# Leo-Li009/fs-dkr

Hardware: AMD Instinct MI355X
Metric: collect() proofs verified/sec at n=64, 2048-bit N; 4096-bit modexp/s/GPU (higher is better)
Workload: dtype u32 (radix-2^29 digits, u64 accumulators); 1 GPU; RefreshMessage::collect n=64 t=32: 60 refresh + 4 JoinMessage, M=256, 2048-bit N (BASELINE configs[2]); one step = the whole collect() call (pack, pre-pass + upload, pipeline, first error, key updates, share recovery); n=64, t=32, refresh=60, joins=4, parallelism=refresh messages sharded over 1 GPU(s)

## Files before the change

### fs-dkr_amd/csrc/capi.cpp

```cpp
#include "fsdkr/fsdkr.h"

#include <hip/hip_runtime.h>

#include <cstdarg>
#include <cstdio>
#include <cstdlib>
#include <cstring>
#include <algorithm>
#include <atomic>
#include <map>
#include <condition_variable>
#include <mutex>
#include <thread>
#include <string>
#include <vector>

#include "ctx.hpp"
#include "kernels.h"
#include "verify.h"

using namespace fsdkr;

namespace fsdkr {

// ... 280 lines not shown
  if (count == 0) return FSDKR_OK;
  uint32_t grp = c->modexp_group ? c->modexp_group : group;
  if (grp == kWideGroup && (group != kWideGroup || k32 != 128)) grp = 16;
  if (grp == kWaveGroup && k32 != 128) grp = 16;
  if (c->ct) grp = 0;
  const bool slide_shape = k32 == 128 ? (grp == 4 || grp == 8 || grp == 16 || grp == kWideGroup)
                                      : (k32 == 192 && grp == 8 && split && split->lo_bit && !split->nadic);
  const bool slide = (desc_flags & kDescSlide) && (desc_flags & kDescOutIdx) && !c->ct && grp == group && slide_shape;
  const int KD = table_digits(k32, grp);
  if (!KD) {
    c->fail("unsupported modulus width %u limbs", k32);
    return FSDKR_E_UNSUPPORTED;
  }
  const uint32_t ebits = exp_bits ? exp_bits : 1;
  const bool nadic = split && split->lo_bit && split->nadic;
  const uint32_t w = nadic ? kNadicWindow : slide ? choose_slide_window(ebits) : choose_window(ebits);
  const uint32_t nwin = (ebits + w - 1) / w;
  const size_t entries = slide ? ((size_t)1 << (w - 1)) + 1 : (size_t)1 << w;
  uint32_t* d_table = (uint32_t*)c->buf(table_tag, sizeof(uint32_t) * (size_t)count * entries * KD);
  if (!d_table) {
    c->fail("device allocation failed (%u instances, window %u)", count, w);
    return FSDKR_E_OOM;
  }
  const size_t n8 = (size_t)count * 8, n4 = (size_t)count * 4;
  ModexpArgs a;
  a.base_ptr = reinterpret_cast<const uint64_t*>(d_desc);
  a.exp_ptr = reinterpret_cast<const uint64_t*>(d_desc + n8);
  a.base_len = reinterpret_cast<const uint32_t*>(d_desc + 2 * n8);
  a.exp_len = reinterpret_cast<const uint32_t*>(d_desc + 2 * n8 + n4);
  a.mod_idx = reinterpret_cast<const uint32_t*>(d_desc + 2 * n8 + 2 * n4);
  a.nwin_i = reinterpret_cast<const uint32_t*>(d_desc + 2 * n8 + 3 * n4);
  a.nwin = nwin;
  a.window = w;
  a.consts = d_consts;
  a.out = d_out;
  a.table = d_table;
  a.count = count;
  a.prio = prio;
  a.group = grp;
  a.ct = c->ct ? 1u : 0u;
  a.slide = slide ? 1u : 0u;
  a.out_idx = (desc_flags & kDescOutIdx) ? reinterpret_cast<const uint32_t*>(d_desc + 2 * n8 + 4 * n4) : nullptr;
  if (split && split->lo_bit) {
    if (!slide || grp != group || !(grp == 4 || grp == 8 || grp == 16 || grp == kWideGroup)) {
      c->fail("split chains need the 4 / 8 / 16 / 32-lane sliding-window shapes, 8 lanes at 192 limbs (group %u)", grp);
      return FSDKR_E_ARG;
    }
    const std::string base(table_tag);
    if (nadic && grp != 16) {
      c->fail("the N-adic head needs the 16-lane shape (group %u)", grp);
      return FSDKR_E_ARG;
    }
    a.nadic = split->nadic;
    a.lo_bit = split->lo_bit;
    a.tail = split->tail ? 1u : 0u;
    a.state = (uint32_t*)c->buf((base + "_state").c_str(), (size_t)count * KD * 4);
    if (!a.state) {
      c->fail("device allocation failed (split chain state)");
      return FSDKR_E_OOM;
    }
    if (split->tail && split->d_desc2) {
      a.base2_ptr = reinterpret_cast<const uint64_t*>(split->d_desc2);
      a.exp2_ptr = reinterpret_cast<const uint64_t*>(split->d_desc2 + n8);
      a.exp2_len = reinterpret_cast<const uint32_t*>(split->d_desc2 + 2 * n8);
      a.table2 = (uint32_t*)c->buf((base + "_t2").c_str(), (size_t)count * 16 * KD * 4);
      if (!a.table2) {
        c->fail("device allocation failed (joint table)");
        return FSDKR_E_OOM;
      }
      if (split->d_desc3) {
        a.base3_ptr = reinterpret_cast<const uint64_t*>(split->d_desc3);
        a.exp3_ptr = reinterpret_cast<const uint64_t*>(split->d_desc3 + n8);
        a.exp3_len = reinterpret_cast<const uint32_t*>(split->d_desc3 + 2 * n8);
        a.exp3_bits = split->exp3_bits;
        a.table3 = (uint32_t*)c->buf((base + "_t3").c_str(), (size_t)count * 16 * KD * 4);
        if (!a.table3) {
          c->fail("device allocation failed (joint table)");
          return FSDKR_E_OOM;
        }
      }
    }
  }
  const size_t tm = c->tbeg("modexp", st);
  int rc = c->hip_check(modexp(k32, a, st), "modexp launch");
  c->tend(tm, st);
  return rc;
}

void ModexpJob::pack(std::vector<uint8_t>& dst) const {
  const size_t n8 = size() * 8, n4 = size() * 4;
  const size_t o = dst.size();
  dst.resize(o + desc_bytes());
  memcpy(dst.data() + o, base_ptr.data(), n8);
  memcpy(dst.data() + o + n8, exp_ptr.data(), n8);
  memcpy(dst.data() + o + 2 * n8, base_len.data(), n4);
  memcpy(dst.data() + o + 2 * n8 + n4, exp_len.data(), n4);
  memcpy(dst.data() + o + 2 * n8 + 2 * n4, mod_idx.data(), n4);
  const uint32_t w = choose_window(exp_bits ? exp_bits : 1);
  uint32_t* nw = reinterpret_cast<uint32_t*>(dst.data() + o + 2 * n8 + 3 * n4);
  for (size_t k = 0; k < size(); ++k) nw[k] = ebits[k] ? (ebits[k] + w - 1) / w : 1u;
  if (!out_idx.empty()) memcpy(dst.data() + o + 2 * n8 + 4 * n4, out_idx.data(), n4);
}

int launch_modexp_job(Ctx* c, const ModexpJob& job, const uint32_t* d_consts, uint32_t* d_out, const char* tag,
                      uint32_t group, uint32_t desc_flags) {
  const uint32_t count = (uint32_t)job.size();
// ... 432 lines not shown
```

### fs-dkr_amd/csrc/collect_prestart.cpp

```cpp
#include "collect.hpp"

namespace fsdkr {

void nadic_consts(const uint32_t* N, uint32_t nl, uint32_t* out) {
  constexpr uint32_t kM29 = (1u << 29) - 1;
  auto digits = [&](const hbn::Limbs& v, uint32_t* dst, int nd) {
    for (int j = 0; j < nd; ++j) {
      const size_t bit = 29u * (size_t)j, w = bit >> 5, sh = bit & 31;
      const uint64_t lo = w < v.size() ? v[w] : 0u, hi = w + 1 < v.size() ? v[w + 1] : 0u;
      dst[j] = (uint32_t)(((hi << 32) | lo) >> sh) & kM29;
    }
  };
  std::fill(out, out + kNadicStride, 0u);
  const hbn::Limbs n = hbn::from(N, nl);
  uint32_t inv = N[0];
  for (int it = 0; it < 5; ++it) inv *= 2u - N[0] * inv;
  const uint32_t k0 = (0u - inv) & kM29;
  const hbn::Limbs Np = hbn::mul(n, hbn::Limbs{k0});
  const hbn::Limbs one{1u};
  hbn::Limbs q, r;
  hbn::divmod_knuth(hbn::mod(hbn::shl(one, 2 * 29 * 72), hbn::mul(Np, Np)), Np, &q, &r);
  const hbn::Limbs nq = q.empty() ? hbn::Limbs{} : hbn::sub(Np, q);
  const hbn::Limbs NN = hbn::mul(n, n);
  const hbn::Limbs C1 = hbn::mod(hbn::shl(one, 3 * 29 * 72), NN);
  const hbn::Limbs C2 = hbn::mod(hbn::mul(hbn::sub(NN, hbn::mod(Np, NN)), C1), NN);
  digits(Np, out + kNadicNp, 72);
  digits(r, out + kNadicR0, 72);
  digits(nq, out + kNadicR1, 72);
  digits(C1, out + kNadicC1, 144);
  digits(C2, out + kNadicC2, 144);
}


static int prestart_fb_tables(Ctx* c, const fsdkr_collect_batch* bs, uint32_t count, GaPre& g, uint32_t n, uint32_t P) {
  if (g.sess.size() != count) return FSDKR_OK;
  const uint32_t M = bs[0].m_security;
  bool exact_s = true, exact_z = true;
  uint32_t nl = 0, Mt = 0, s1l = 0, s3l = 0, zl = 0;
  for (uint32_t k = 0; k < count; ++k) {
    const fsdkr_collect_batch* b = bs + k;
    if (!b->recv_ntilde || !b->recv_h1 || !b->recv_h2 || !b->s1l || !b->s3l || !b->ped_T || !b->ped_N || !b->zl ||
        !b->m_security || b->m_security != M)
      return FSDKR_OK;
    exact_s = exact_s && b->pdl_s1 && b->pdl_s3 && b->rp_s1 && b->rp_s2;
    exact_z = exact_z && b->ped_Z;
    nl = std::max(nl, b->nl);
    Mt += b->n_refresh + b->n_join;
    s1l = std::max(s1l, b->s1l);
    s3l = std::max(s3l, b->s3l);
    zl = std::max(zl, b->zl);
    for (uint32_t i = 0; i < g.sess[k].n; ++i)
      if (!is_odd(b->recv_ntilde + (size_t)i * b->nl)) return FSDKR_OK;
  }
  uint32_t bh1 = 1, bh2 = 1, bz = 1;
  if (exact_s) {
    for (uint32_t k = 0; k < count; ++k) {
      const fsdkr_collect_batch* b = bs + k;
      for (size_t p = 0; p < (size_t)g.sess[k].R * g.sess[k].n; ++p) {
        bh1 = std::max(bh1, std::max(hbn::bitlen(b->pdl_s1 + p * b->s1l, b->s1l), hbn::bitlen(b->rp_s1 + p * b->s1l, b->s1l)));
        bh2 = std::max(bh2, std::max(hbn::bitlen(b->pdl_s3 + p * b->s3l, b->s3l), hbn::bitlen(b->rp_s2 + p * b->s3l, b->s3l)));
      }
    }
  } else {
    bh1 = 32 * s1l;
    bh2 = 32 * s3l;
  }
  if (exact_z) {
    for (uint32_t k = 0; k < count; ++k) {
      const fsdkr_collect_batch* b = bs + k;
      const size_t rows = (size_t)(b->n_refresh + b->n_join) * M;
      for (size_t q = 0; q < rows; ++q) bz = std::max(bz, hbn::bitlen(b->ped_Z + q * b->zl, b->zl));
    }
  } else {
    bz = 32 * zl;
  }
  const uint32_t w = fb_window(std::max(std::max(bh1, bh2), bz));
  const FbLayout L = fb_layout(n, Mt, w, bh1, bh2, bz);
  const uint32_t nb = 2 * n + Mt, entries = L.entries, nmod = n + Mt;
  const int KD = shape_digits(nl);
  std::vector<uint32_t> bbits(nb), bcnt(nb, M);
  for (uint32_t r = 0; r < n; ++r) {
    bbits[r] = bh1;
    bbits[n + Mt + r] = bh2;
// ... 672 lines not shown
```

### fs-dkr_amd/csrc/kernels.h

```cpp
#pragma once
#include <hip/hip_runtime.h>
#include <stdint.h>

namespace fsdkr {

constexpr int BLOCK = 256;

constexpr int cons_stride(int kd) { return 6 * kd + 8; }
constexpr int cons_scaled(int kd) { return 3 * kd + 4; }
constexpr bool scaled_ok(int kd, int k32) { return 32 * k32 + 31 <= 29 * kd; }

struct ModexpArgs {
  const uint64_t* base_ptr;
  const uint32_t* base_len;
  const uint64_t* exp_ptr;
  const uint32_t* exp_len;
  uint32_t nwin;
  uint32_t window;
  const uint32_t* nwin_i;
  const uint32_t* mod_idx;
  const uint32_t* consts;
  uint32_t* out;
  uint32_t* table;
  uint32_t count;
  uint32_t prio;
  uint32_t group;
  uint32_t ct;
  uint32_t slide;
  const uint32_t* out_idx;
  uint32_t lo_bit = 0;
  uint32_t tail = 0;
  uint32_t* state = nullptr;
  const uint64_t* base2_ptr = nullptr;
  const uint64_t* exp2_ptr = nullptr;
  const uint32_t* exp2_len = nullptr;
  uint32_t* table2 = nullptr;
  const uint32_t* nadic = nullptr;
  const uint64_t* base3_ptr = nullptr;
  const uint64_t* exp3_ptr = nullptr;
  const uint32_t* exp3_len = nullptr;
  uint32_t* table3 = nullptr;
  uint32_t exp3_bits = 0;
};

constexpr int kNadicNp = 0, kNadicR0 = 72, kNadicR1 = 144, kNadicC1 = 216, kNadicC2 = 360, kNadicStride = 512;
constexpr uint32_t kNadicWindow = 7;

int shape_digits(uint32_t k32);
constexpr uint32_t kWideGroup = 32;
constexpr uint32_t kWaveGroup = 64;
int shape_digits_g(uint32_t k32, uint32_t group);
int table_digits(uint32_t k32, uint32_t group);
hipError_t mod_setup(uint32_t k32, const uint32_t* mods, uint32_t n_mod, uint32_t* consts, hipStream_t st);
hipError_t mod_setup_wave(uint32_t k32, const uint32_t* mods, uint32_t n_mod, uint32_t* consts, hipStream_t st);
hipError_t mod_setup_g(uint32_t k32, uint32_t group, const uint32_t* mods, uint32_t n_mod, uint32_t* consts,
                       hipStream_t st);
hipError_t modexp(uint32_t k32, const ModexpArgs& a, hipStream_t st);

struct MrTailArgs {
  const uint32_t* x;
  const uint32_t* consts;
  const uint32_t* s;
  uint32_t s_max;
  uint32_t* verdict;
  uint32_t count;
};
constexpr uint32_t kPrimeLimbs = 32;
hipError_t mr_tail(uint32_t k32, const MrTailArgs& a, hipStream_t st);

}
```

### fs-dkr_amd/csrc/modexp.hip

```cpp
#include "mont29.hpp"
#include "kernels.h"
#include <cstdlib>
#include <initializer_list>

namespace fsdkr {

template <int KD, int G, int K32>
__global__ __launch_bounds__(BLOCK) void mod_setup_kernel(const uint32_t* __restrict__ mods, uint32_t n_mod,
                                                          uint32_t* __restrict__ consts) {
  using MT = Mont29<KD, G>;
  constexpr int L = MT::L;
  constexpr int IPB = BLOCK / G;
  constexpr bool SC = scaled_ok(KD, K32);
  __shared__ uint32_t lds[IPB * KD];
  const int g = threadIdx.x % G;
  const int li = threadIdx.x / G;
  const uint32_t mi = blockIdx.x * IPB + li;
  if (mi >= (SC ? 2 * n_mod : n_mod)) return;
  const bool scaled = SC && mi >= n_mod;
  const uint32_t m = scaled ? mi - n_mod : mi;
  __builtin_amdgcn_s_setprio(3);
  uint32_t* stream = lds + li * KD;
  const uint32_t* N = mods + (size_t)m * K32;
  MT M;
// ... 398 lines not shown
  constexpr int IPB = BLOCK / G;
  __shared__ uint32_t lds[IPB * KD];
  const int g = threadIdx.x % G;
  const int li = threadIdx.x / G;
  const uint32_t inst = blockIdx.x * (blockDim.x / G) + li;
  if (inst >= a.count) return;
  if (a.prio == 1) __builtin_amdgcn_s_setprio(1);
  else if (a.prio == 2) __builtin_amdgcn_s_setprio(2);
  else if (a.prio >= 3) __builtin_amdgcn_s_setprio(3);
  uint32_t* stream = lds + li * KD;
  const uint32_t* C = a.nadic + (size_t)a.mod_idx[inst] * kNadicStride;
  const bool hi = g >= 8;
  uint32_t sh_hi = hi ? 1u : 0u, m_hi = hi ? 0xFFFFFFFFu : 0u;
  asm volatile("" : "+v"(sh_hi), "+v"(m_hi));
  MT M;
  M.init_pair(g);
#pragma unroll
  for (int j = 0; j < L; ++j) M.n[j] = C[kNadicNp + (g & 7) * L + j];
  M.ninv = 1u;
  const uint32_t tw = 1u << (kNadicWindow - 1);
  uint32_t* T = a.table + (size_t)inst * (tw + 1) * KD;
  const uint64_t ea = a.exp_ptr[inst];
  const uint32_t* E = reinterpret_cast<const uint32_t*>(
      ((uint64_t)(uint32_t)__builtin_amdgcn_readfirstlane((int)(uint32_t)(ea >> 32)) << 32) |
      (uint32_t)__builtin_amdgcn_readfirstlane((int)(uint32_t)ea));
  const int exp_limbs = __builtin_amdgcn_readfirstlane((int)a.exp_len[inst]);
  auto bit = [&](int i) -> uint32_t { return (E[i >> 5] >> (i & 31)) & 1u; };
  int top = 32 * exp_limbs - 1;
  while (top >= 0 && E[top >> 5] == 0) top = (top & ~31) - 1;
  while (top >= 0 && !bit(top)) --top;
  const int lo = (int)a.lo_bit;
  auto window = [&](int i, int* jl) -> uint32_t {
    int j = max(i - (int)kNadicWindow + 1, lo);
    while (!bit(j)) ++j;
    uint32_t d = 0;
    for (int k = i; k >= j; --k) d = (d << 1) | bit(k);
    *jl = j;
    return d;
  };
  uint32_t acc[L];
#pragma unroll
  for (int j = 0; j < L; ++j) acc[j] = 0u;
  const uint32_t* B = reinterpret_cast<const uint32_t*>(a.base_ptr[inst]);
  const int blen = (int)min(a.base_len[inst], 64u);
  auto load = [&](const uint32_t* row) {
#pragma unroll
    for (int j = 0; j < L; ++j) acc[j] = row[g * L + j];
  };
  auto store = [&](uint32_t* row) {
#pragma unroll
    for (int j = 0; j < L; ++j) row[g * L + j] = acc[j];
  };
  const bool none = top < lo;
  {
    uint32_t b[L];
    __builtin_amdgcn_wave_barrier();
#pragma unroll
    for (int j = 0; j < L; ++j) {
      const int d = g * L + j;
      b[j] = C[kNadicR0 + d];
      if (!hi) stream[d] = none ? (d == 0 ? 1u : 0u) : digit_of(B, blen, d);
    }
    __builtin_amdgcn_wave_barrier();
    M.product_pair(acc, b, stream);
  }
  auto square = [&]() {
    __builtin_amdgcn_wave_barrier();
    lds_put<KD, G>(stream, acc, g);
    __builtin_amdgcn_wave_barrier();
    uint32_t b[L];
#pragma unroll
    for (int j = 0; j < L; ++j) b[j] = acc[j] << sh_hi;
    M.product_pair(acc, b, stream);
  };
  if (!none) {
    store(T);
    square();
    store(T + (size_t)tw * KD);
    load(T);
    int phase = tw > 1 ? 2 : 3, i = top, pend_mul = -1;
    uint32_t jt = 1, pend_sq = 0;
    for (;;) {
      if (phase == 3) {
        if (i == top) {
          int jl;
          const uint32_t d = window(i, &jl);
          load(T + (size_t)(d >> 1) * KD);
          i = jl - 1;
        }
        if (pend_sq == 0 && pend_mul < 0)
          while (i >= lo && !bit(i)) {
            ++pend_sq;
            --i;
          }
        for (; pend_sq; --pend_sq) square();
      }
      const uint32_t* src;
      if (phase == 2) {
        src = T + (size_t)tw * KD;
      } else if (pend_mul >= 0) {
        src = T + (size_t)pend_mul * KD;
        pend_mul = -1;
      } else if (i < lo) {
        break;
      } else {
        int jl;
        const uint32_t d = window(i, &jl);
        pend_sq = (uint32_t)(i - jl + 1);
        pend_mul = (int)(d >> 1);
        i = jl - 1;
        continue;
      }
      uint32_t y[L];
      __builtin_amdgcn_wave_barrier();
#pragma unroll
      for (int j = 0; j < L; ++j) y[j] = src[g * L + j];
      if (!hi) {
#pragma unroll
        for (int j = 0; j < L; ++j) {
          stream[g * L + j] = y[j];
          stream[72 + g * L + j] = acc[j];
        }
      }
#pragma unroll
      for (int j = 0; j < L; ++j) y[j] &= m_hi;
      __builtin_amdgcn_wave_barrier();
      M.product_pair2(acc, acc, y, stream, stream + 72);
      if (phase == 2) {
        store(T + (size_t)jt * KD);
        if (++jt == tw) phase = 3;
      }
    }
  }
#pragma unroll
  for (int j = 0; j < L; ++j) a.state[(size_t)inst * KD + g * L + j] = acc[j];
}

template <int KD, int G, int K32, bool QS, bool NA = false, bool J3 = false>
__global__ __launch_bounds__(BLOCK, 2) void modexp_tail_kernel(const ModexpArgs a) {
  using MT = Mont29<KD, G>;
  constexpr int L = MT::L;
  constexpr int IPB = BLOCK / G;
  constexpr int STRIDE = cons_stride(KD);
  static_assert(!QS || scaled_ok(KD, K32), "quotient-scaled chains: N' within R/4");
  __shared__ uint32_t lds[IPB * KD];
  const int g = threadIdx.x % G;
  const int li = threadIdx.x / G;
  const uint32_t inst = blockIdx.x * (blockDim.x / G) + li;
  if (inst >= a.count) return;
  if (a.prio == 1) __builtin_amdgcn_s_setprio(1);
  else if (a.prio == 2) __builtin_amdgcn_s_setprio(2);
  else if (a.prio >= 3) __builtin_amdgcn_s_setprio(3);
  uint32_t* stream = lds + li * KD;
  const uint32_t* C0 = a.consts + (size_t)a.mod_idx[inst] * STRIDE;
  const uint32_t* C = QS ? C0 + cons_scaled(KD) : C0;
  MT M;
  M.init_lane(g);
#pragma unroll
  for (int j = 0; j < L; ++j) M.n[j] = C[g * L + j];
  M.ninv = C[3 * KD];
  auto mulx = [&](uint32_t* x) {
    if constexpr (QS) M.mul_s(x, x, stream);
    else M.mul(x, x, stream);
  };
  const uint32_t w = a.window, tw = 1u << (w - 1);
  uint32_t* T = a.table + (size_t)inst * (tw + 1) * KD;
  const uint64_t ea = a.exp_ptr[inst];
  const uint32_t* E = reinterpret_cast<const uint32_t*>(
      ((uint64_t)(uint32_t)__builtin_amdgcn_readfirstlane((int)(uint32_t)(ea >> 32)) << 32) |
      (uint32_t)__builtin_amdgcn_readfirstlane((int)(uint32_t)ea));
  const int exp_limbs = __builtin_amdgcn_readfirstlane((int)a.exp_len[inst]);
  auto bit = [&](int i) -> uint32_t { return (i >> 5) < exp_limbs ? (E[i >> 5] >> (i & 31)) & 1u : 0u; };
  const int lo = (int)a.lo_bit;
  constexpr bool ACC_LATE = K32 > 128;
  static_assert(!(ACC_LATE && NA), "the N-adic entry converts the accumulator first");
  uint32_t acc[L];
  if constexpr (!ACC_LATE) {
#pragma unroll
    for (int j = 0; j < L; ++j) acc[j] = a.state[(size_t)inst * KD + g * L + j];
  }
  auto put_row = [&](const uint32_t* row) {
    __builtin_amdgcn_wave_barrier();
#pragma unroll
    for (int j = 0; j < L; ++j) stream[g * L + j] = row[g * L + j];
// ... 123 lines not shown
      pend_d = d;
    }
    __builtin_amdgcn_wave_barrier();
    lds_put<KD, G>(stream, acc, g);
    __builtin_amdgcn_wave_barrier();
    if constexpr (QS) M.sqr_s(acc, acc, stream);
    else M.sqr(acc, acc, stream);
    if (!NA && i == pend_at) {
      put_row(T + (size_t)(pend_d >> 1) * KD);
      mulx(acc);
      pend_at = -1;
    }
    if (NA && (i & 3) == 0) {
      const uint32_t d = (i >> 5) < exp_limbs ? (E[i >> 5] >> (i & 31)) & 15u : 0u;
      if (d) {
        put_row(T + (size_t)d * KD);
        mulx(acc);
      }
    }
    if (joint && (i & 3) == 0) {
      put_row(T2 + (size_t)((ew >> (i & 31)) & 15u) * KD);
      mulx(acc);
    }
    if constexpr (J3) {
      if ((i & 3) == 0 && i < e3bits) {
        put_row(T3 + (size_t)((ew3 >> (i & 31)) & 15u) * KD);
        mulx(acc);
      }
    }
  }
  if constexpr (QS) {
    const uint32_t* CX = C0;
    if constexpr (ACC_LATE) asm volatile("" : "+v"(CX) : "v"(acc[0]));
#pragma unroll
    for (int j = 0; j < L; ++j) M.n[j] = CX[g * L + j];
    M.ninv = CX[3 * KD];
  }
  __builtin_amdgcn_wave_barrier();
#pragma unroll
  for (int j = 0; j < L; ++j) stream[g * L + j] = (g == 0 && j == 0) ? 1u : 0u;
  __builtin_amdgcn_wave_barrier();
  M.mul(acc, acc, stream);
  M.carry_exact(acc);
  M.sub_if_ge(acc);
  __builtin_amdgcn_wave_barrier();
  lds_put<KD, G>(stream, acc, g);
  __builtin_amdgcn_wave_barrier();
  uint32_t* O = a.out + (size_t)(a.out_idx ? a.out_idx[inst] : inst) * K32;
  constexpr int LO = K32 / G;
#pragma unroll
  for (int k = 0; k < LO; ++k) O[g * LO + k] = limb_of(stream, KD, g * LO + k);
}

template <int KR, int L, int K32>
__global__ __launch_bounds__(64) void modexp_wave_kernel(const ModexpArgs a) {
  constexpr int KD = 64 * L;
  using MT = Mont29<KD, 64, KR>;
  constexpr int STRIDE = cons_stride(KR);
  __shared__ uint32_t lds[KD];
  const int g = threadIdx.x;
  const uint32_t inst = blockIdx.x;
  if (inst >= a.count) return;
  if (a.prio == 1) __builtin_amdgcn_s_setprio(1);
  else if (a.prio == 2) __builtin_amdgcn_s_setprio(2);
  else if (a.prio >= 3) __builtin_amdgcn_s_setprio(3);
  const uint32_t* C = a.consts + (size_t)a.mod_idx[inst] * STRIDE;
  const bool live = g * L < KR;
  MT M;
  M.init_lane(g);
#pragma unroll
  for (int j = 0; j < L; ++j) M.n[j] = live ? C[g * L + j] : 0u;
  M.ninv = (uint32_t)__builtin_amdgcn_readfirstlane((int)C[3 * KR]);
  const uint32_t w = a.window;
  const uint32_t tsize = 1u << w;
  uint32_t* T = a.table + (size_t)inst * tsize * KD;
  const uint32_t* E = reinterpret_cast<const uint32_t*>(a.exp_ptr[inst]);
  const uint32_t exp_limbs = a.exp_len[inst];
  uint32_t acc[L], opnd[L];
  const uint32_t* B = reinterpret_cast<const uint32_t*>(a.base_ptr[inst]);
  const int blen = (int)min(a.base_len[inst], (uint32_t)K32);
#pragma unroll
  for (int j = 0; j < L; ++j) acc[j] = digit_of(B, blen, g * L + j);
#pragma unroll
  for (int j = 0; j < L; ++j) T[g * L + j] = live ? C[KR + g * L + j] : 0u;
  const uint32_t nwin = a.nwin_i ? max(1u, a.nwin_i[inst]) : a.nwin;
  auto digit = [&](uint32_t k) -> uint32_t {
    const uint32_t p = (nwin - 1 - k) * w;
    const uint32_t lo = p >> 5, sh = p & 31;
    const uint32_t v0 = (lo < exp_limbs) ? E[lo] : 0u;
    const uint32_t v1 = (lo + 1 < exp_limbs) ? E[lo + 1] : 0u;
    return (uint32_t)(mk64(v0, v1) >> sh) & (tsize - 1);
  };
  const uint32_t n_build = tsize - 1;
  const uint32_t n_steps = n_build + (nwin - 1) * (w + 1) + 1;
  uint32_t k = 1, sub = 0;
  for (uint32_t st = 0; st < n_steps; ++st) {
    if (st == n_build) {
      const uint32_t d0 = digit(0);
#pragma unroll
      for (int j = 0; j < L; ++j) acc[j] = T[(size_t)d0 * KD + g * L + j];
    }
    if (st >= n_build && st < n_steps - 1 && sub < w) {
      M.sqr_w(acc, acc);
    } else {
      const uint32_t* src = (st == 0) ? nullptr : (st < n_build) ? T + KD : (st == n_steps - 1) ? nullptr
                                                                            : T + (size_t)digit(k) * KD;
// ... 22 lines not shown
  __builtin_amdgcn_wave_barrier();
  uint32_t* O = a.out + (size_t)(a.out_idx ? a.out_idx[inst] : inst) * K32;
  for (int q = g; q < K32; q += 64) O[q] = limb_of(lds, KR, q);
}

template <int KR, int L, int K32>
static hipError_t launch_setup_wave(const uint32_t* mods, uint32_t n_mod, uint32_t* consts, hipStream_t st) {
  const uint32_t waves = scaled_ok(KR, K32) ? 2 * n_mod : n_mod;
  if (waves == 0) return hipSuccess;
  hipLaunchKernelGGL((mod_setup_wave_kernel<KR, L, K32>), dim3(waves), dim3(64), 0, st, mods, n_mod, consts);
  return hipGetLastError();
}
template <int KD, int G, int K32>
static hipError_t launch_setup(const uint32_t* mods, uint32_t n_mod, uint32_t* consts, hipStream_t st) {
  constexpr int IPB = BLOCK / G;
  const uint32_t inst = scaled_ok(KD, K32) ? 2 * n_mod : n_mod;
  const uint32_t blocks = (inst + IPB - 1) / IPB;
  if (blocks == 0) return hipSuccess;
  hipLaunchKernelGGL((mod_setup_kernel<KD, G, K32>), dim3(blocks), dim3(BLOCK), 0, st, mods, n_mod, consts);
  return hipGetLastError();
}
constexpr uint32_t kSmallLaunchLanes = 256u * 4u * 64u;
static inline uint32_t block_threads(uint32_t lanes) { return lanes <= kSmallLaunchLanes ? 64u : (uint32_t)BLOCK; }

template <int KD, int G, int K32, bool CT = false, bool QS = false>
static hipError_t launch_modexp(const ModexpArgs& a, hipStream_t st) {
  const uint32_t bs = block_threads(a.count * G);
  const uint32_t ipb = bs / G;
  const uint32_t blocks = (a.count + ipb - 1) / ipb;
  if (blocks == 0) return hipSuccess;
  hipLaunchKernelGGL((modexp_kernel<KD, G, K32, CT, QS>), dim3(blocks), dim3(bs), 0, st, a);
  return hipGetLastError();
}

template <int KD, int G, int K32, bool QS>
static hipError_t launch_modexp_slide(const ModexpArgs& a, hipStream_t st) {
  const uint32_t bs = block_threads(a.count * G);
  const uint32_t ipb = bs / G;
  const uint32_t blocks = (a.count + ipb - 1) / ipb;
  if (blocks == 0) return hipSuccess;
  hipLaunchKernelGGL((modexp_slide_kernel<KD, G, K32, QS>), dim3(blocks), dim3(bs), 0, st, a);
  return hipGetLastError();
}

static hipError_t launch_modexp_nadic_head(const ModexpArgs& a, hipStream_t st) {
  const uint32_t bs = block_threads(a.count * 16);
  const uint32_t ipb = bs / 16;
  const uint32_t blocks = (a.count + ipb - 1) / ipb;
  if (blocks == 0) return hipSuccess;
  hipLaunchKernelGGL(modexp_nadic_head_kernel, dim3(blocks), dim3(bs), 0, st, a);
  return hipGetLastError();
}

template <int KD, int G, int K32, bool QS, bool NA = false, bool J3 = false>
static hipError_t launch_modexp_tail(const ModexpArgs& a, hipStream_t st) {
  const uint32_t bs = block_threads(a.count * G);
  const uint32_t ipb = bs / G;
  const uint32_t blocks = (a.count + ipb - 1) / ipb;
  if (blocks == 0) return hipSuccess;
  hipLaunchKernelGGL((modexp_tail_kernel<KD, G, K32, QS, NA, J3>), dim3(blocks), dim3(bs), 0, st, a);
  return hipGetLastError();
}

template <int KR, int L, int K32>
static hipError_t launch_modexp_wave(const ModexpArgs& a, hipStream_t st) {
  if (a.count == 0) return hipSuccess;
  hipLaunchKernelGGL((modexp_wave_kernel<KR, L, K32>), dim3(a.count), dim3(64), 0, st, a);
  return hipGetLastError();
}

hipError_t mod_setup_wave(uint32_t k32, const uint32_t* mods, uint32_t n_mod, uint32_t* consts, hipStream_t st) {
  if (k32 == 96) return launch_setup_wave<108, 2, 96>(mods, n_mod, consts, st);
  return mod_setup(k32, mods, n_mod, consts, st);
}

int shape_digits(uint32_t k32) {
  switch (k32) {
    case 64: return 72;
    case 96: return 108;
    case 128: return 144;
    case 192: return 216;
    default: return 0;
  }
}

int shape_digits_g(uint32_t k32, uint32_t group) {
  if (k32 == kPrimeLimbs) return 36;
  return (k32 == 128 && group == kWideGroup) ? 160 : shape_digits(k32);
}

int table_digits(uint32_t k32, uint32_t group) {
  if (k32 == 128 && group == kWaveGroup) return 192;
  return shape_digits_g(k32, group);
}

hipError_t mod_setup_g(uint32_t k32, uint32_t group, const uint32_t* mods, uint32_t n_mod, uint32_t* consts,
                       hipStream_t st) {
  if (k32 == 128 && group == kWideGroup) return launch_setup<160, 8, 128>(mods, n_mod, consts, st);
  return mod_setup(k32, mods, n_mod, consts, st);
}

hipError_t mod_setup(uint32_t k32, const uint32_t* mods, uint32_t n_mod, uint32_t* consts, hipStream_t st) {
  switch (k32) {
    case 32: return launch_setup<36, 2, 32>(mods, n_mod, consts, st);
    case 64: return launch_setup<72, 8, 64>(mods, n_mod, consts, st);
    case 96: return launch_setup<108, 4, 96>(mods, n_mod, consts, st);
// ... 7 lines not shown
  for (int g : allowed)
    if (g == forced) return g;
  constexpr uint64_t kLaneCapacity = 256ull * 4 * 3 * 64;
  int best = min_auto;
  for (int g : allowed)
    if (g > best && (uint64_t)count * (uint64_t)g <= kLaneCapacity) best = g;
  return best;
}

hipError_t modexp(uint32_t k32, const ModexpArgs& a, hipStream_t st) {
  if (a.ct) {
    if (a.group == kWideGroup) return hipErrorInvalidValue;
    switch (k32) {
      case 32: return launch_modexp<36, 4, 32, true>(a, st);
      case 64: return launch_modexp<72, 8, 64, true>(a, st);
      case 96: return launch_modexp<108, 4, 96, true>(a, st);
      case 128: return launch_modexp<144, 8, 128, true>(a, st);
      case 192: return launch_modexp<216, 8, 192, true>(a, st);
      default: return hipErrorInvalidValue;
    }
  }
  if (a.slide && k32 == 192) {
    if (a.ct || a.group != 8 || !a.lo_bit || a.nadic || !a.state) return hipErrorInvalidValue;
    if (!a.tail) return launch_modexp_slide<216, 8, 192, true>(a, st);
    if (a.base3_ptr) {
      if (!a.base2_ptr || !a.exp3_ptr || !a.exp3_len || !a.table3 || (a.exp3_bits & 3u) || a.exp3_bits > a.lo_bit)
        return hipErrorInvalidValue;
      return launch_modexp_tail<216, 8, 192, true, false, true>(a, st);
    }
    return launch_modexp_tail<216, 8, 192, true>(a, st);
  }
  if (a.slide) {
    if (k32 != 128 || a.ct || a.group == kWaveGroup) return hipErrorInvalidValue;
    if (a.base3_ptr) {
      if (!a.lo_bit || !a.tail || a.nadic || !a.base2_ptr || !a.exp3_ptr || !a.exp3_len || !a.table3 ||
          (a.exp3_bits & 3u) || a.exp3_bits > a.lo_bit)
        return hipErrorInvalidValue;
      switch (a.group) {
        case kWideGroup: return launch_modexp_tail<160, 32, 128, true, false, true>(a, st);
        case 16: return launch_modexp_tail<144, 16, 128, true, false, true>(a, st);
        case 8: return launch_modexp_tail<144, 8, 128, true, false, true>(a, st);
        case 4: return launch_modexp_tail<144, 4, 128, true, false, true>(a, st);
        default: return hipErrorInvalidValue;
      }
    }
    if (a.group == kWideGroup) {
      if (a.lo_bit && a.tail)
        return launch_modexp_tail<160, 32, 128, true>(a, st);
      return launch_modexp_slide<160, 32, 128, true>(a, st);
    }
    if (a.lo_bit) {
      if (a.nadic) {
        if (a.group != 16 || a.window != kNadicWindow || !a.state) return hipErrorInvalidValue;
        return a.tail ? launch_modexp_tail<144, 16, 128, true, true>(a, st) : launch_modexp_nadic_head(a, st);
      }
      switch (a.group) {
        case 16: return a.tail ? launch_modexp_tail<144, 16, 128, true>(a, st)
                               : launch_modexp_slide<144, 16, 128, true>(a, st);
        case 8: return a.tail ? launch_modexp_tail<144, 8, 128, true>(a, st)
                              : launch_modexp_slide<144, 8, 128, true>(a, st);
        case 4: return a.tail ? launch_modexp_tail<144, 4, 128, true>(a, st)
                              : launch_modexp_slide<144, 4, 128, true>(a, st);
        default: return hipErrorInvalidValue;
      }
    }
    switch (pick_group(a.count, (int)a.group, {4, 8, 16}, 4)) {
      case 16: return launch_modexp_slide<144, 16, 128, true>(a, st);
      case 8: return launch_modexp_slide<144, 8, 128, true>(a, st);
      default: return launch_modexp_slide<144, 4, 128, true>(a, st);
    }
  }
  switch (k32) {
    case 32:
      return pick_group(a.count, (int)a.group, {2, 4}, 4) == 2 ? launch_modexp<36, 2, 32>(a, st)
                                                              : launch_modexp<36, 4, 32>(a, st);
    case 64:
      switch (pick_group(a.count, (int)a.group, {2, 4, 8}, 4)) {
        case 8: return launch_modexp<72, 8, 64, false, true>(a, st);
        case 4: return launch_modexp<72, 4, 64, false, true>(a, st);
        default: return launch_modexp<72, 2, 64>(a, st);
      }
    case 96: return launch_modexp<108, 4, 96, false, true>(a, st);
    case 128:
      if (a.group == kWideGroup)
        return launch_modexp<160, 32, 128, false, true>(a, st);
      if (a.group == kWaveGroup) return launch_modexp_wave<144, 3, 128>(a, st);
      switch (pick_group(a.count, (int)a.group, {4, 8, 16}, 4)) {
        case 16: return launch_modexp<144, 16, 128, false, true>(a, st);
        case 8: return launch_modexp<144, 8, 128, false, true>(a, st);
        default: return launch_modexp<144, 4, 128, false, true>(a, st);
      }
    case 192:
      if (pick_group(a.count, (int)a.group, {4, 8}, 4) == 8)
        return launch_modexp<216, 8, 192, false, true>(a, st);
      return launch_modexp<216, 4, 192, false, true>(a, st);
    default: return hipErrorInvalidValue;
  }
}

}
```

### fs-dkr_amd/fsdkr/_native.py

```python
import ctypes
import os

import numpy as np

_HERE = os.path.dirname(os.path.abspath(__file__))
LIB_PATH = os.environ.get("FSDKR_LIB") or os.path.join(_HERE, "libfsdkr.so")

FSDKR_OK = 0
FSDKR_E_ARG = -1
FSDKR_E_HIP = -2
FSDKR_E_OOM = -3
FSDKR_E_UNSUPPORTED = -4
FSDKR_CFG_TIMING = 1
FSDKR_CFG_FB_BGMW = 2
FSDKR_CFG_FB_COMB = 4
FSDKR_CFG_INV_EACH = 8
FSDKR_CFG_GA_FULLWIDTH = 16

u32p = ctypes.POINTER(ctypes.c_uint32)


class FsdkrError(RuntimeError):
    def __init__(self, code, msg):
        super().__init__(f"fsdkr error {code}: {msg}")
        self.code = code


class _Cfg(ctypes.Structure):
    _fields_ = [("device", ctypes.c_int32), ("flags", ctypes.c_uint32)]


class CollectBatchC(ctypes.Structure):
    _fields_ = [(f, ctypes.c_uint32) for f in ("n_refresh", "n_join", "t", "m_security", "key_bits", "nl",
                                               "s1l", "s3l", "el", "zl", "yl")] + \
               [(f, u32p) for f in ("party_index", "msg_lens", "recv_n", "recv_ntilde", "recv_h1", "recv_h2",
                                    "enc", "commit", "pdl_z", "pdl_u3", "pdl_s2", "pdl_u1", "pdl_u2", "pdl_s1",
                                    "pdl_s3", "rp_z", "rp_s", "rp_e", "rp_s1", "rp_s2", "vss", "ped_S", "ped_T",
                                    "ped_N", "ped_A", "ped_Z", "ck_n", "ck_sigma", "dlog_N", "dlog_g", "dlog_ni",
                                    "dlog_x1", "dlog_x2", "dlog_y1", "dlog_y2")] + [("n_recv", ctypes.c_uint32)] + \
               [("vss_len", u32p), ("range_lens", u32p), ("ckl", ctypes.c_uint32), ("recv_avail", ctypes.c_uint32),
                ("ped_lens", u32p), ("ck_lens", u32p), ("pdl_s3_neg", ctypes.POINTER(ctypes.c_uint8)),
                ("neg_bits", ctypes.POINTER(ctypes.c_uint8)), ("ped_a_neg", ctypes.POINTER(ctypes.c_uint8))]


u8p = ctypes.POINTER(ctypes.c_uint8)


class VerdictsC(ctypes.Structure):
    _fields_ = [(f, u8p) for f in ("feldman", "pdl", "range", "ped", "ck", "dlog")] + \
               [(f, ctypes.c_uint32) for f in ("cap_pairs", "cap_msgs", "cap_joins")]


class BobBatchC(ctypes.Structure):
    _fields_ = [(f, ctypes.c_uint32) for f in ("count", "n_keys", "nl", "el", "s1l", "s2l", "t1l", "t2l")] + \
               [(f, u32p) for f in ("N", "Ntilde", "h1", "h2", "key_idx", "a_enc", "mta", "z", "t", "s", "e",
                                    "s1", "s2", "t1", "t2", "X", "u")]


class RecoverJobC(ctypes.Structure):
    _fields_ = [("nl", ctypes.c_uint32), ("t_vss", ctypes.c_uint32), ("t_key", ctypes.c_uint32),
                ("n_new", ctypes.c_uint32), ("old_index", u32p), ("cts", u32p), ("p", u32p), ("q", u32p),
                ("points", u32p), ("flags", ctypes.c_uint32)]


class RecoveredC(ctypes.Structure):
    _fields_ = [("share", ctypes.c_uint32 * 8), ("y", ctypes.c_uint32 * 16), ("pk_vec", u32p),
                ("status", ctypes.c_int32)]


def _struct_dtype(cls):
# ... 630 lines not shown
```

### include/fsdkr/fsdkr.h

```cpp
#ifndef FSDKR_FSDKR_H
#define FSDKR_FSDKR_H

#include <stdint.h>

#ifdef __cplusplus
extern "C" {
#endif

#define FSDKR_OK 0
#define FSDKR_E_ARG (-1)
#define FSDKR_E_HIP (-2)
#define FSDKR_E_OOM (-3)
#define FSDKR_E_UNSUPPORTED (-4)

typedef struct fsdkr_ctx fsdkr_ctx;

typedef struct fsdkr_cfg {
  int32_t device;
  uint32_t flags;
} fsdkr_cfg;

#define FSDKR_CFG_TIMING 1u
#define FSDKR_CFG_FB_BGMW 2u
#define FSDKR_CFG_FB_COMB 4u
#define FSDKR_CFG_INV_EACH 8u
#define FSDKR_CFG_GA_FULLWIDTH 16u

int fsdkr_ctx_create(const fsdkr_cfg* cfg, fsdkr_ctx** out);
void fsdkr_ctx_destroy(fsdkr_ctx* ctx);
const char* fsdkr_last_error(const fsdkr_ctx* ctx);
int fsdkr_ctx_set_modexp_group(fsdkr_ctx* ctx, uint32_t lanes);
int fsdkr_ctx_set_timing(fsdkr_ctx* ctx, int on);
int fsdkr_ctx_set_flags(fsdkr_ctx* ctx, uint32_t flags);

int fsdkr_ctx_set_cu_split(fsdkr_ctx* ctx, uint32_t ga_cus);
int fsdkr_device_available(void);

int fsdkr_modexp_batch(fsdkr_ctx* ctx, uint32_t mod_limbs, uint32_t count, const uint32_t* base,
                       const uint32_t* exp, uint32_t exp_limbs, const uint32_t* mod_idx,
                       const uint32_t* mods, uint32_t n_mod, uint32_t* out);

int fsdkr_modexp_batch_ct(fsdkr_ctx* ctx, uint32_t mod_limbs, uint32_t count, const uint32_t* base,
                          const uint32_t* exp, uint32_t exp_limbs, const uint32_t* mod_idx,
                          const uint32_t* mods, uint32_t n_mod, uint32_t* out);

int fsdkr_mod_inverse(fsdkr_ctx* ctx, uint32_t mod_limbs, uint32_t count, const uint32_t* y, const uint32_t* m,
                      uint32_t* out, uint32_t* unit);

int fsdkr_modexp_batch_device(fsdkr_ctx* ctx, uint32_t mod_limbs, uint32_t count, const uint32_t* d_base,
                              const uint32_t* d_exp, uint32_t exp_limbs, uint32_t exp_bits,
                              const uint32_t* d_mod_idx, const uint32_t* d_mods, uint32_t n_mod,
                              uint32_t* d_out);

int fsdkr_modexp_keyed_device(fsdkr_ctx* ctx, uint32_t mod_limbs, uint32_t count, const uint32_t* d_base,
                              const uint32_t* d_exp, uint32_t exp_limbs, uint32_t exp_bits,
                              const uint32_t* d_mod_idx, const uint32_t* d_mods, uint32_t n_mod,
                              uint32_t* d_out);

int fsdkr_miller_rabin(fsdkr_ctx* ctx, uint32_t mod_limbs, uint32_t count, const uint32_t* cand,
                       const uint32_t* bases, uint32_t* verdict);


typedef struct fsdkr_collect_batch {
  uint32_t n_refresh;
  uint32_t n_join;
  uint32_t t;
  uint32_t m_security;
  uint32_t key_bits;
  uint32_t nl;
  uint32_t s1l, s3l, el, zl, yl;
  const uint32_t* party_index;
  const uint32_t* msg_lens;
  const uint32_t *recv_n, *recv_ntilde, *recv_h1, *recv_h2;
  const uint32_t* enc;
  const uint32_t* commit;
  const uint32_t *pdl_z, *pdl_u3, *pdl_s2;
  const uint32_t* pdl_u1;
  const uint32_t* pdl_u2;
  const uint32_t* pdl_s1;
// ... 204 lines not shown
```

Measured before the change: 204,100 proofs/s.

## Run N-adic split-chain tail in paired half-width Montgomery arithmetic

```diff
diff --git a/fs-dkr_amd/csrc/capi.cpp b/fs-dkr_amd/csrc/capi.cpp
--- a/fs-dkr_amd/csrc/capi.cpp
+++ b/fs-dkr_amd/csrc/capi.cpp
@@ -356,6 +356,7 @@
       return FSDKR_E_ARG;
     }
     a.nadic = split->nadic;
+    a.nadic_tail_full = (c->flags & FSDKR_CFG_GA_TAIL_FULLWIDTH) ? 1u : 0u;
     a.lo_bit = split->lo_bit;
     a.tail = split->tail ? 1u : 0u;
     a.state = (uint32_t*)c->buf((base + "_state").c_str(), (size_t)count * KD * 4);
diff --git a/fs-dkr_amd/csrc/collect_prestart.cpp b/fs-dkr_amd/csrc/collect_prestart.cpp
--- a/fs-dkr_amd/csrc/collect_prestart.cpp
+++ b/fs-dkr_amd/csrc/collect_prestart.cpp
@@ -29,6 +29,10 @@
   digits(nq, out + kNadicR1, 72);
   digits(C1, out + kNadicC1, 144);
   digits(C2, out + kNadicC2, 144);
+  hbn::Limbs q2, r2;
+  hbn::divmod_knuth(hbn::mod(hbn::shl(one, 2048 + 2 * 29 * 72), hbn::mul(Np, Np)), Np, &q2, &r2);
+  digits(r2, out + kNadicP2, 72);
+  digits(q2.empty() ? hbn::Limbs{} : hbn::sub(Np, q2), out + kNadicP2 + 72, 72);
 }
 
 
diff --git a/fs-dkr_amd/csrc/kernels.h b/fs-dkr_amd/csrc/kernels.h
--- a/fs-dkr_amd/csrc/kernels.h
+++ b/fs-dkr_amd/csrc/kernels.h
@@ -41,9 +41,11 @@
   const uint32_t* exp3_len = nullptr;
   uint32_t* table3 = nullptr;
   uint32_t exp3_bits = 0;
+  uint32_t nadic_tail_full = 0;
 };
 
-constexpr int kNadicNp = 0, kNadicR0 = 72, kNadicR1 = 144, kNadicC1 = 216, kNadicC2 = 360, kNadicStride = 512;
+constexpr int kNadicNp = 0, kNadicR0 = 72, kNadicR1 = 144, kNadicC1 = 216, kNadicC2 = 360, kNadicP2 = 504,
+              kNadicStride = 656;
 constexpr uint32_t kNadicWindow = 7;
 
 int shape_digits(uint32_t k32);
diff --git a/fs-dkr_amd/csrc/modexp.hip b/fs-dkr_amd/csrc/modexp.hip
--- a/fs-dkr_amd/csrc/modexp.hip
+++ b/fs-dkr_amd/csrc/modexp.hip
@@ -474,17 +474,18 @@
     for (int j = 0; j < L; ++j) row[g * L + j] = acc[j];
   };
   const bool none = top < lo;
-  {
+  for (int pass = none ? 0 : 1; pass < 2; ++pass) {
     uint32_t b[L];
     __builtin_amdgcn_wave_barrier();
 #pragma unroll
     for (int j = 0; j < L; ++j) {
       const int d = g * L + j;
       b[j] = C[kNadicR0 + d];
-      if (!hi) stream[d] = none ? (d == 0 ? 1u : 0u) : digit_of(B, blen, d);
+      if (!hi) stream[d] = pass == 0 ? (d == 0 ? 1u : 0u) : digit_of(B, blen, d);
     }
     __builtin_amdgcn_wave_barrier();
     M.product_pair(acc, b, stream);
+    if (pass == 0) store(a.state + (size_t)inst * KD);
   }
   auto square = [&]() {
     __builtin_amdgcn_wave_barrier();
@@ -495,63 +496,62 @@
     for (int j = 0; j < L; ++j) b[j] = acc[j] << sh_hi;
     M.product_pair(acc, b, stream);
   };
-  if (!none) {
-    store(T);
-    square();
-    store(T + (size_t)tw * KD);
-    load(T);
-    int phase = tw > 1 ? 2 : 3, i = top, pend_mul = -1;
-    uint32_t jt = 1, pend_sq = 0;
-    for (;;) {
-      if (phase == 3) {
-        if (i == top) {
-          int jl;
-          const uint32_t d = window(i, &jl);
-          load(T + (size_t)(d >> 1) * KD);
-          i = jl - 1;
-        }
-        if (pend_sq == 0 && pend_mul < 0)
-          while (i >= lo && !bit(i)) {
-            ++pend_sq;
-            --i;
-          }
-        for (; pend_sq; --pend_sq) square();
-      }
-      const uint32_t* src;
-      if (phase == 2) {
-        src = T + (size_t)tw * KD;
-      } else if (pend_mul >= 0) {
-        src = T + (size_t)pend_mul * KD;
-        pend_mul = -1;
-      } else if (i < lo) {
-        break;
-      } else {
+  store(T);
+  square();
+  store(T + (size_t)tw * KD);
+  load(T);
+  int phase = tw > 1 ? 2 : 3, i = top, pend_mul = -1;
+  uint32_t jt = 1, pend_sq = 0;
+  for (;;) {
+    if (phase == 3) {
+      if (none) return;
+      if (i == top) {
         int jl;
         const uint32_t d = window(i, &jl);
-        pend_sq = (uint32_t)(i - jl + 1);
-        pend_mul = (int)(d >> 1);
+        load(T + (size_t)(d >> 1) * KD);
         i = jl - 1;
-        continue;
-      }
-      uint32_t y[L];
-      __builtin_amdgcn_wave_barrier();
-#pragma unroll
-      for (int j = 0; j < L; ++j) y[j] = src[g * L + j];
-      if (!hi) {
-#pragma unroll
-        for (int j = 0; j < L; ++j) {
-          stream[g * L + j] = y[j];
-          stream[72 + g * L + j] = acc[j];
+      }
+      if (pend_sq == 0 && pend_mul < 0)
+        while (i >= lo && !bit(i)) {
+          ++pend_sq;
+          --i;
         }
-      }
-#pragma unroll
-      for (int j = 0; j < L; ++j) y[j] &= m_hi;
-      __builtin_amdgcn_wave_barrier();
-      M.product_pair2(acc, acc, y, stream, stream + 72);
-      if (phase == 2) {
-        store(T + (size_t)jt * KD);
-        if (++jt == tw) phase = 3;
-      }
+      for (; pend_sq; --pend_sq) square();
+    }
+    const uint32_t* src;
+    if (phase == 2) {
+      src = T + (size_t)tw * KD;
+    } else if (pend_mul >= 0) {
+      src = T + (size_t)pend_mul * KD;
+      pend_mul = -1;
+    } else if (i < lo) {
+      break;
+    } else {
+      int jl;
+      const uint32_t d = window(i, &jl);
+      pend_sq = (uint32_t)(i - jl + 1);
+      pend_mul = (int)(d >> 1);
+      i = jl - 1;
+      continue;
+    }
+    uint32_t y[L];
+    __builtin_amdgcn_wave_barrier();
+#pragma unroll
+    for (int j = 0; j < L; ++j) y[j] = src[g * L + j];
+    if (!hi) {
+#pragma unroll
+      for (int j = 0; j < L; ++j) {
+        stream[g * L + j] = y[j];
+        stream[72 + g * L + j] = acc[j];
+      }
+    }
+#pragma unroll
+    for (int j = 0; j < L; ++j) y[j] &= m_hi;
+    __builtin_amdgcn_wave_barrier();
+    M.product_pair2(acc, acc, y, stream, stream + 72);
+    if (phase == 2) {
+      store(T + (size_t)jt * KD);
+      if (++jt == tw) phase = 3;
     }
   }
 #pragma unroll
@@ -781,6 +781,179 @@
   for (int k = 0; k < LO; ++k) O[g * LO + k] = limb_of(stream, KD, g * LO + k);
 }
 
+__global__ __launch_bounds__(BLOCK) void modexp_nadic_tail_kernel(const ModexpArgs a) {
+  using MT = Mont29<72, 8>;
+  constexpr int L = MT::L, KD = 144, G = 16, K32 = 128;
+  constexpr int IPB = BLOCK / G;
+  __shared__ uint32_t lds[IPB * KD];
+  const int g = threadIdx.x % G;
+  const int li = threadIdx.x / G;
+  const uint32_t inst = blockIdx.x * (blockDim.x / G) + li;
+  if (inst >= a.count) return;
+  if (a.prio == 1) __builtin_amdgcn_s_setprio(1);
+  else if (a.prio == 2) __builtin_amdgcn_s_setprio(2);
+  else if (a.prio >= 3) __builtin_amdgcn_s_setprio(3);
+  uint32_t* stream = lds + li * KD;
+  const uint32_t* CN = a.nadic + (size_t)a.mod_idx[inst] * kNadicStride;
+  const bool hi = g >= 8;
+  uint32_t sh_hi = hi ? 1u : 0u, m_hi = hi ? 0xFFFFFFFFu : 0u;
+  asm volatile("" : "+v"(sh_hi), "+v"(m_hi));
+  MT M;
+  M.init_pair(g);
+#pragma unroll
+  for (int j = 0; j < L; ++j) M.n[j] = CN[kNadicNp + (g & 7) * L + j];
+  M.ninv = 1u;
+  const uint32_t tw = 1u << (kNadicWindow - 1);
+  const uint32_t* T = a.table + (size_t)inst * (tw + 1) * KD;
+  const uint64_t ea = a.exp_ptr[inst];
+  const uint32_t* E = reinterpret_cast<const uint32_t*>(
+      ((uint64_t)(uint32_t)__builtin_amdgcn_readfirstlane((int)(uint32_t)(ea >> 32)) << 32) |
+      (uint32_t)__builtin_amdgcn_readfirstlane((int)(uint32_t)ea));
+  const int exp_limbs = __builtin_amdgcn_readfirstlane((int)a.exp_len[inst]);
+  auto bit = [&](int i) -> uint32_t { return (i >> 5) < exp_limbs ? (E[i >> 5] >> (i & 31)) & 1u : 0u; };
+  const int lo = (int)a.lo_bit;
+  uint32_t acc[L];
+  auto square = [&]() {
+    __builtin_amdgcn_wave_barrier();
+    lds_put<KD, G>(stream, acc, g);
+    __builtin_amdgcn_wave_barrier();
+    uint32_t b[L];
+#pragma unroll
+    for (int j = 0; j < L; ++j) b[j] = acc[j] << sh_hi;
+    M.product_pair(acc, b, stream);
+  };
+  auto times = [&](const uint32_t* src) {
+    uint32_t y[L];
+    __builtin_amdgcn_wave_barrier();
+#pragma unroll
+    for (int j = 0; j < L; ++j) y[j] = src[g * L + j];
+    if (!hi) {
+#pragma unroll
+      for (int j = 0; j < L; ++j) {
+        stream[g * L + j] = y[j];
+        stream[72 + g * L + j] = acc[j];
+      }
+    }
+#pragma unroll
+    for (int j = 0; j < L; ++j) y[j] &= m_hi;
+    __builtin_amdgcn_wave_barrier();
+    M.product_pair2(acc, acc, y, stream, stream + 72);
+  };
+  const bool joint = a.base2_ptr != nullptr;
+  uint32_t* T2 = joint ? a.table2 + (size_t)inst * 16 * KD : nullptr;
+  const uint32_t* E2 = nullptr;
+  uint32_t e2len = 0;
+  if (joint) {
+    E2 = reinterpret_cast<const uint32_t*>(a.exp2_ptr[inst]);
+    e2len = a.exp2_len[inst];
+    const uint32_t* B2 = reinterpret_cast<const uint32_t*>(a.base2_ptr[inst]);
+    uint32_t b[L], b2[L];
+    __builtin_amdgcn_wave_barrier();
+#pragma unroll
+    for (int j = 0; j < L; ++j) {
+      const int d = g * L + j;
+      b[j] = CN[kNadicR0 + d];
+      b2[j] = CN[kNadicP2 + d];
+      if (!hi) stream[d] = d == 0 ? 1u : 0u;
+    }
+    __builtin_amdgcn_wave_barrier();
+    M.product_pair(acc, b, stream);
+#pragma unroll
+    for (int j = 0; j < L; ++j) T2[g * L + j] = acc[j];
+    __builtin_amdgcn_wave_barrier();
+#pragma unroll
+    for (int j = 0; j < L; ++j)
+      stream[g * L + j] = digit_of(B2 + (hi ? 64 : 0), 64, (g & 7) * L + j);
+    __builtin_amdgcn_wave_barrier();
+    M.product_pair2(acc, b, b2, stream, stream + 72);
+#pragma unroll
+    for (int j = 0; j < L; ++j) T2[KD + g * L + j] = acc[j];
+    __builtin_amdgcn_wave_barrier();
+#pragma unroll
+    for (int j = 0; j < L; ++j) {
+      if (!hi) stream[g * L + j] = acc[j];
+      b[j] = acc[j] & m_hi;
+    }
+    for (int u = 2; u < 16; ++u) {
+      __builtin_amdgcn_wave_barrier();
+      if (!hi) {
+#pragma unroll
+        for (int j = 0; j < L; ++j) stream[72 + g * L + j] = acc[j];
+      }
+      __builtin_amdgcn_wave_barrier();
+      M.product_pair2(acc, acc, b, stream, stream + 72);
+#pragma unroll
+      for (int j = 0; j < L; ++j) T2[(size_t)u * KD + g * L + j] = acc[j];
+    }
+  }
+#pragma unroll
+  for (int j = 0; j < L; ++j) acc[j] = a.state[(size_t)inst * KD + g * L + j];
+  int pend_at = -1;
+  uint32_t pend_d = 0, ew = 0;
+  for (int i = lo - 1; i >= 0; --i) {
+    if ((i & 31) == 31 && joint) ew = ((uint32_t)(i >> 5) < e2len) ? E2[i >> 5] : 0u;
+    if (pend_at < 0 && bit(i)) {
+      int j = max(i - (int)kNadicWindow + 1, 0);
+      while (!bit(j)) ++j;
+      uint32_t d = 0;
+      for (int k = i; k >= j; --k) d = (d << 1) | bit(k);
+      pend_at = j;
+      pend_d = d;
+    }
+    square();
+    if (i == pend_at) {
+      times(T + (size_t)(pend_d >> 1) * KD);
+      pend_at = -1;
+    }
+    if (joint && (i & 3) == 0) times(T2 + (size_t)((ew >> (i & 31)) & 15u) * KD);
+  }
+  using MF = Mont29<KD, G>;
+  static_assert(MF::L == L, "pair and full-width rows hold 9 digits per lane");
+  const uint32_t* C0 = a.consts + (size_t)a.mod_idx[inst] * cons_stride(KD);
+  const uint32_t* C = C0 + cons_scaled(KD);
+  MF F;
+  F.init_lane(g);
+#pragma unroll
+  for (int j = 0; j < L; ++j) F.n[j] = C[g * L + j];
+  F.ninv = C[3 * KD];
+  uint32_t y[L];
+  __builtin_amdgcn_wave_barrier();
+#pragma unroll
+  for (int j = 0; j < L; ++j) {
+    stream[g * L + j] = g < 8 ? acc[j] : 0u;
+    y[j] = CN[kNadicC1 + g * L + j];
+  }
+  __builtin_amdgcn_wave_barrier();
+  F.mul_s(y, y, stream);
+  __builtin_amdgcn_wave_barrier();
+#pragma unroll
+  for (int j = 0; j < L; ++j) stream[(g ^ 8) * L + j] = g >= 8 ? acc[j] : 0u;
+#pragma unroll
+  for (int j = 0; j < L; ++j) acc[j] = CN[kNadicC2 + g * L + j];
+  __builtin_amdgcn_wave_barrier();
+  F.mul_s(acc, acc, stream);
+#pragma unroll
+  for (int j = 0; j < L; ++j) acc[j] += y[j];
+  F.carry_exact(acc);
+#pragma unroll
+  for (int j = 0; j < L; ++j) F.n[j] = C0[g * L + j];
+  F.ninv = C0[3 * KD];
+  __builtin_amdgcn_wave_barrier();
+#pragma unroll
+  for (int j = 0; j < L; ++j) stream[g * L + j] = (g == 0 && j == 0) ? 1u : 0u;
+  __builtin_amdgcn_wave_barrier();
+  F.mul(acc, acc, stream);
+  F.carry_exact(acc);
+  F.sub_if_ge(acc);
+  __builtin_amdgcn_wave_barrier();
+  lds_put<KD, G>(stream, acc, g);
+  __builtin_amdgcn_wave_barrier();
+  uint32_t* O = a.out + (size_t)(a.out_idx ? a.out_idx[inst] : inst) * K32;
+  constexpr int LO = K32 / G;
+#pragma unroll
+  for (int k = 0; k < LO; ++k) O[g * LO + k] = limb_of(stream, KD, g * LO + k);
+}
+
 template <int KR, int L, int K32>
 __global__ __launch_bounds__(64) void modexp_wave_kernel(const ModexpArgs a) {
   constexpr int KD = 64 * L;
@@ -909,6 +1082,15 @@
   return hipGetLastError();
 }
 
+static hipError_t launch_modexp_nadic_tail(const ModexpArgs& a, hipStream_t st) {
+  const uint32_t bs = block_threads(a.count * 16);
+  const uint32_t ipb = bs / 16;
+  const uint32_t blocks = (a.count + ipb - 1) / ipb;
+  if (blocks == 0) return hipSuccess;
+  hipLaunchKernelGGL(modexp_nadic_tail_kernel, dim3(blocks), dim3(bs), 0, st, a);
+  return hipGetLastError();
+}
+
 template <int KD, int G, int K32, bool QS, bool NA = false, bool J3 = false>
 static hipError_t launch_modexp_tail(const ModexpArgs& a, hipStream_t st) {
   const uint32_t bs = block_threads(a.count * G);
@@ -1022,7 +1204,8 @@
     if (a.lo_bit) {
       if (a.nadic) {
         if (a.group != 16 || a.window != kNadicWindow || !a.state) return hipErrorInvalidValue;
-        return a.tail ? launch_modexp_tail<144, 16, 128, true, true>(a, st) : launch_modexp_nadic_head(a, st);
+        if (!a.tail) return launch_modexp_nadic_head(a, st);
+        return a.nadic_tail_full ? launch_modexp_tail<144, 16, 128, true, true>(a, st) : launch_modexp_nadic_tail(a, st);
       }
       switch (a.group) {
         case 16: return a.tail ? launch_modexp_tail<144, 16, 128, true>(a, st)
diff --git a/fs-dkr_amd/fsdkr/_native.py b/fs-dkr_amd/fsdkr/_native.py
--- a/fs-dkr_amd/fsdkr/_native.py
+++ b/fs-dkr_amd/fsdkr/_native.py
@@ -16,6 +16,7 @@
 FSDKR_CFG_FB_COMB = 4
 FSDKR_CFG_INV_EACH = 8
 FSDKR_CFG_GA_FULLWIDTH = 16
+FSDKR_CFG_GA_TAIL_FULLWIDTH = 32
 
 u32p = ctypes.POINTER(ctypes.c_uint32)
 
diff --git a/include/fsdkr/fsdkr.h b/include/fsdkr/fsdkr.h
--- a/include/fsdkr/fsdkr.h
+++ b/include/fsdkr/fsdkr.h
@@ -25,6 +25,7 @@
 #define FSDKR_CFG_FB_COMB 4u
 #define FSDKR_CFG_INV_EACH 8u
 #define FSDKR_CFG_GA_FULLWIDTH 16u
+#define FSDKR_CFG_GA_TAIL_FULLWIDTH 32u
 
 int fsdkr_ctx_create(const fsdkr_cfg* cfg, fsdkr_ctx** out);
 void fsdkr_ctx_destroy(fsdkr_ctx* ctx);
```

New measurement: 210,100 proofs/s (median of 6 runs). 1.03x the previous value.
